# soham2560/MPCHoloNavigation

Measured on AMD Instinct MI355X. Metric: rollouts/sec per computeVelocityCommands() tick, higher is better.
Workload: dtype f32

## Files before the change

### mpcholonavigation_amd/csrc/smpc_lane.hip

```cpp

#include <hip/hip_runtime.h>
#include <stdint.h>
#include <stdio.h>

#include <type_traits>

#include "smpc_dev.h"
#include "smpc_device_math.h"
#include "smpc_tail.h"
#include "smpc_lane_common.h"
#include "smpc_inst.h"

#ifndef WAVE
#define WAVE 64
#endif
#ifndef LANE_X_RR_NOLOAD
#define LANE_X_RR_NOLOAD 0
#endif
#define LANE_BLOCK 512
#ifndef LANE_BLOCK_RR
#define LANE_BLOCK_RR 512
#endif

#ifndef LANE_X_GAMMA_N
#define LANE_X_GAMMA_N 0
#endif
#ifndef LANE_X_GAMMA_UC
#define LANE_X_GAMMA_UC 1
#endif
#ifndef LANE_X_FURTHEST_WINDOW
#define LANE_X_FURTHEST_WINDOW 1
#endif
#ifndef LANE_X_PFW_MIN
#define LANE_X_PFW_MIN 1
#endif
#ifndef LANE_X_CELL_AX
#define LANE_X_CELL_AX 1
#endif
#ifndef LANE_X_PIN_LDS
#define LANE_X_PIN_LDS 0
#endif
#ifndef LANE_X_PARK_STEP
#define LANE_X_PARK_STEP 0
#endif
#ifndef LANE_X_CONST_VGPR
#define LANE_X_CONST_VGPR 0
#endif

template <bool TO_GM>
__global__ void __launch_bounds__(256) smpc_relayout(const float* __restrict__ src, float* __restrict__ dst,
                                                    uint32_t B, uint32_t T)
{
  __shared__ float tile[32][33];
  const uint32_t b0 = blockIdx.x * 32, t0 = blockIdx.y * 32;
  const uint32_t lx = threadIdx.x & 31, ly = threadIdx.x >> 5;
  if (TO_GM) {
    for (uint32_t k = ly; k < 32; k += 8) {
      const uint32_t b = b0 + k, t = t0 + lx;
      tile[k][lx] = (b < B && t < T) ? src[(size_t)b * T + t] : 0.f;
    }
    __syncthreads();
    for (uint32_t k = ly; k < 32; k += 8) {
      const uint32_t t = t0 + k, b = b0 + lx;
      if (b < B && t < T) dst[SMPC_GM_INDEX(b, t, T)] = tile[lx][k];
    }
  } else {
    for (uint32_t k = ly; k < 32; k += 8) {
      const uint32_t t = t0 + k, b = b0 + lx;
      tile[lx][k] = (b < B && t < T) ? src[SMPC_GM_INDEX(b, t, T)] : 0.f;
    }
    __syncthreads();
    for (uint32_t k = ly; k < 32; k += 8) {
      const uint32_t b = b0 + k, t = t0 + lx;
      if (b < B && t < T) dst[(size_t)b * T + t] = tile[k][lx];
    }
  }
}

hipError_t smpc_launch_relayout(const float* src, float* dst, uint32_t B, uint32_t T, bool to_gm, hipStream_t st)
{
  const dim3 grid((B + 31) / 32, (T + 31) / 32);
  if (to_gm) hipLaunchKernelGGL(smpc_relayout<true>, grid, dim3(256), 0, st, src, dst, B, T);
  else hipLaunchKernelGGL(smpc_relayout<false>, grid, dim3(256), 0, st, src, dst, B, T);
  return hipGetLastError();
}

__global__ void __launch_bounds__(64) smpc_lane_reduce_kernel(const float* __restrict__ v,
                                                              const float* __restrict__ w,
                                                              float* __restrict__ out)
{
  const int lane = threadIdx.x;
  float V[64];
#pragma unroll
  for (int t = 0; t < 64; ++t) V[t] = v[lane * 64 + t];
  const LaneW lw = lane_weights(w[lane], lane);
  out[lane] = lane_reduce64(V, lw, lane);
}

hipError_t smpc_launch_lane_reduce(const float* v, const float* w, float* out, hipStream_t st)
{
  hipLaunchKernelGGL(smpc_lane_reduce_kernel, dim3(1), dim3(64), 0, st, v, w, out);
  return hipGetLastError();
}

#define LANE_PASS_KERNEL smpc_pass_lane
#define LANE_PASS_POW false
#include "smpc_lane_pass.inc"
#undef LANE_PASS_KERNEL
#undef LANE_PASS_POW
#define LANE_PASS_KERNEL smpc_pass_lane_pow
#define LANE_PASS_POW true
#include "smpc_lane_pass.inc"
#undef LANE_PASS_KERNEL
#undef LANE_PASS_POW

#define LANE_INST(...) {__VA_ARGS__, reinterpret_cast<const void*>(&smpc_pass_lane<__VA_ARGS__>), false}
#define LANE_INST_POW(...) {__VA_ARGS__, reinterpret_cast<const void*>(&smpc_pass_lane_pow<__VA_ARGS__>), true}
static const LaneInst kLaneInst[] = {
  LANE_INST(false, false, false, 1, false, false, false, 0, false),
  LANE_INST(true, false, false, 1, false, false, true, 0, false),
  LANE_INST(false, true, false, 1, false, false, false, 0, false),
  LANE_INST(true, true, false, 1, false, false, true, 0, false),
  LANE_INST(false, true, false, 1, false, false, true, 0, false),
  LANE_INST(false, true, false, 1, false, false, true, 56, false),
  LANE_INST(false, false, true, 1, false, false, false, 0, false),
  LANE_INST(true, false, true, 1, false, false, true, 0, false),
  LANE_INST(false, true, true, 1, false, false, false, 0, false),
  LANE_INST(true, true, true, 1, false, false, true, 0, false),
  LANE_INST(true, true, false, 1, true, false, true, 0, false),
  LANE_INST(true, true, false, 2, true, false, true, 0, false),
  LANE_INST(false, true, false, 1, false, true, false, 0, false),
  LANE_INST(true, true, false, 1, false, true, true, 0, false),
  LANE_INST(true, true, false, 1, false, false, true, 0, true),
  LANE_INST(false, true, false, 1, false, false, true, 56, true),
  LANE_INST(true, true, true, 1, false, false, true, 0, true),
  LANE_INST(false, true, true, 1, false, false, true, 56, true),
  LANE_INST_POW(true, true, false, 1, false, false, true, 0, false),
  LANE_INST_POW(false, true, false, 1, false, false, true, 0, false),
  LANE_INST_POW(false, true, false, 1, false, false, true, 56, false),
  LANE_INST_POW(false, true, false, 1, false, false, false, 0, false),
  LANE_INST_POW(true, true, false, 1, false, true, true, 0, false),
  LANE_INST_POW(false, true, false, 1, false, true, false, 0, false),
  LANE_INST_POW(true, false, false, 1, false, false, true, 0, false),
  LANE_INST_POW(false, false, false, 1, false, false, false, 0, false),
};
#undef LANE_INST
#undef LANE_INST_POW

static const LaneInst* lane_find(bool full, bool obst, bool many, int nch, bool rr, bool ga, bool quads, int tc, bool dep,
                                 bool pow = false)
{
  for (const LaneInst& k : kLaneInst)
    if (k.full == full && k.obst == obst && k.many == many && k.nch == nch && k.rr == rr && k.ga == ga &&
        k.quads == quads && k.tc == tc && k.dep == dep && k.pow == pow)
      return &k;
  return nullptr;
}

const LaneInst* lane_select(uint32_t flags, uint32_t T, bool rr, bool many, float acker_r, bool pow)
{
  const uint32_t dep_set = SD_CONSTRAINT | SD_COST | SD_TWIRLING, lean_extra = dep_set | SD_GOAL | SD_PATH_ANGLE;
  if (flags & (SD_STORE_TRAJ | SD_USE_PATH_YAW | (SD_EXTRA_CRITICS & ~lean_extra))) return nullptr;
  const bool obst = (flags & (SD_OBSTACLES | SD_COST)) != 0;
  const bool full = T == 64u;
  if (pow) {
    if (rr || many || T > 64u || (flags & lean_extra)) return nullptr;
    if (flags & SD_GOAL_ANGLE) return obst ? lane_find(full, true, false, 1, false, true, full, 0, false, true) : nullptr;
    if (obst && T == 56u) return lane_find(false, true, false, 1, false, false, true, 56, false, true);
    return lane_find(full, obst, false, 1, false, false, full || (obst && (T & 3u) == 0u), 0, false, true);
  }
  if (rr) {
    if (!(flags & SD_OBSTACLES) || (flags & (lean_extra | SD_GOAL_ANGLE)) || (T != 64u && T != 128u)) return nullptr;
    return lane_find(true, true, many, T > 64u ? 2 : 1, true, false, true, 0, false);
  }
  if (T > 64u) return nullptr;
  if (flags & dep_set) {
    if (!obst || (flags & (SD_GOAL_ANGLE | SD_GOAL)) || ((flags & SD_COST) && (flags & SD_OBSTACLES)) ||
        acker_r >= 0.f || (!full && T != 56u))
      return nullptr;
    return lane_find(full, true, many, 1, false, false, true, full ? 0 : 56, true);
  }
  if (flags & (SD_GOAL | SD_PATH_ANGLE)) return nullptr;
  if (flags & SD_GOAL_ANGLE)
    return obst ? lane_find(full, true, many, 1, false, true, full, 0, false) : nullptr;
  if (many) return lane_find(full, obst, true, 1, false, false, full, 0, false);
  if (obst && T == 56u) return lane_find(false, true, false, 1, false, false, true, 56, false);
  return lane_find(full, obst, false, 1, false, false, full || (obst && (T & 3u) == 0u), 0, false);
}

const LaneInst* lane_occupancy_row(uint32_t T, bool rr)
{
  if (rr) return lane_find(true, true, false, T > 64u ? 2 : 1, true, false, true, 0, false);
  return lane_find(T == 64u, true, false, 1, false, false, T == 64u, 0, false);
}

hipError_t lane_launch(const LaneInst* k, const SmpcDev& p, const SmpcDev* d_many, uint32_t n, const SmpcLds& L,
                       uint32_t grid, uint32_t block, hipStream_t st)
{
  if (!k || k->many != (d_many != nullptr)) return hipErrorInvalidValue;
  if (k->rr ? block != LANE_BLOCK_RR : (block != LANE_BLOCK && block != LANE_BLOCK / 2)) return hipErrorInvalidValue;
  auto b = [](bool v) {return v ? "true" : "false";};
  snprintf(smpc_last_pass_kernel, sizeof(smpc_last_pass_kernel), "smpc_pass_lane%s<%s, %s, %s, %d, %s, %s, %s, %d, %s>",
           k->pow ? "_pow" : "", b(k->full), b(k->obst), b(k->many), k->nch, b(k->rr), b(k->ga), b(k->quads), k->tc, b(k->dep));
  static const SmpcDev none{};
  void* args[] = {const_cast<SmpcDev*>(d_many ? &none : &p), const_cast<SmpcLds*>(&L), &d_many};
  return inst_launch(k->fn, d_many ? dim3(grid, n) : dim3(grid), block, args, L.total, st);
}

uint32_t smpc_lane_block() {return LANE_BLOCK;}
uint32_t smpc_lane_block_rr() {return LANE_BLOCK_RR;}

hipError_t lane_set_lds_limit(int bytes) {return inst_set_lds_limit(kLaneInst, bytes);}
```

### mpcholonavigation_amd/csrc/smpc_lane_common.h

```cpp
#ifndef SMPC_LANE_COMMON_H_
#define SMPC_LANE_COMMON_H_

#include <hip/hip_runtime.h>
#include <stdint.h>

#include "smpc_dev.h"
#include "smpc_device_math.h"

#ifndef WAVE
#define WAVE 64
#endif

typedef unsigned u32x2 __attribute__((ext_vector_type(2)));
typedef const float __attribute__((address_space(4))) * cfloat_p;
typedef float f32x32 __attribute__((ext_vector_type(32)));
typedef float f32x4 __attribute__((ext_vector_type(4)));
typedef float f32x2 __attribute__((ext_vector_type(2)));
#define LANE_PARK_STRIDE 68

struct LaneW {
  float wa, wb;
};

#define SMPC_DPP_NODE(NAME, CTRL, BANKS)                                                    \
  __device__ __forceinline__ float NAME(float a, float b)                                   \
  {                                                                                         \
    float t;                                                                                \
    asm("s_nop 1\n\t"                                                              \
                 "v_add_f32_dpp %0, %1, %1 " CTRL " row_mask:0xf bank_mask:0xf\n\t"         \
                 "v_add_f32_dpp %0, %2, %2 " CTRL " row_mask:0xf bank_mask:" BANKS          \
                 : "=&v"(t)                                                                 \
                 : "v"(a), "v"(b));                                                         \
    return t;                                                                               \
  }
SMPC_DPP_NODE(node_bit3, "row_ror:8", "0xc")
SMPC_DPP_NODE(node_bit2, "row_half_mirror", "0xa")

template <int CTRL>
__device__ __forceinline__ float dpp_mov(float v)
{
  return __uint_as_float(
    (uint32_t)__builtin_amdgcn_update_dpp(0, (int)__float_as_uint(v), CTRL, 0xF, 0xF, false));
}

template <int K, int Rr>
__device__ __forceinline__ float lane_reduce_node(const float (&V)[64], const LaneW& w, int lane)
{
  if constexpr (K == 0) {
    return V[Rr];
  } else {
    const float a = lane_reduce_node<K - 1, Rr>(V, w, lane);
    const float b = lane_reduce_node<K - 1, Rr + (64 >> K)>(V, w, lane);
    if constexpr (K == 1) {
      const u32x2 s = __builtin_amdgcn_permlane32_swap(__float_as_uint(a), __float_as_uint(b),
                                                       false, false);
      return fmaf(w.wa, __uint_as_float(s.x), w.wb * __uint_as_float(s.y));
    } else if constexpr (K == 2) {
      const u32x2 s = __builtin_amdgcn_permlane16_swap(__float_as_uint(a), __float_as_uint(b),
                                                       false, false);
      return __uint_as_float(s.x) + __uint_as_float(s.y);
    } else if constexpr (K == 3) {
      return node_bit3(a, b);
    } else if constexpr (K == 4) {
      return node_bit2(a, b);
    } else if constexpr (K == 5) {
      const float ta = a + dpp_mov<0x4E>(a);
      const float tb = b + dpp_mov<0x4E>(b);
      return (lane & 2) ? tb : ta;
    } else {
      const float ta = a + dpp_mov<0xB1>(a);
      const float tb = b + dpp_mov<0xB1>(b);
      return (lane & 1) ? tb : ta;
    }
  }
}

__device__ __forceinline__ LaneW lane_weights(float w, int lane)
{
  const float wo = __shfl_xor(w, 32, WAVE);
  LaneW r;
  r.wa = lane < 32 ? w : wo;
  r.wb = lane < 32 ? wo : w;
  return r;
}

__device__ __forceinline__ float lane_reduce64(const float (&V)[64], const LaneW& w, int lane)
{
  return lane_reduce_node<6, 0>(V, w, lane);
}

__device__ __forceinline__ int cvt_floor_i32(float q)
{
  int r;
  asm("v_cvt_flr_i32_f32 %0, %1" : "=v"(r) : "v"(q));
  return r;
}

__device__ __forceinline__ uint32_t cell_byte_exact(const SmpcDev& p, uint8_t* s_map, float x,
                                                    float y, uint32_t slot)
{
  const uint32_t nwin = (uint32_t)(p.win_w * p.win_h);
  uint32_t mx = 0, my = 0;
  bool on = cell_index_exact((double)x, p.ox, p.res, p.W, mx);
  on = cell_index_exact((double)y, p.oy, p.res, p.H, my) && on;
  if (!on) return nwin;
  const uint32_t wx = mx - (uint32_t)p.win_x0, wy = my - (uint32_t)p.win_y0;
  if (wx < (uint32_t)p.win_w && wy < (uint32_t)p.win_h) return wy * p.win_w + wx;
  s_map[nwin + 1 + slot] = p.map[(size_t)my * p.W + mx];
  return nwin + 1 + slot;
}

#endif
```

### mpcholonavigation_amd/csrc/smpc_lane_pass.inc

```
template <bool FULL, bool OBST, bool MANY, int NCH, bool RR, bool GA = false, bool QUADS = FULL, int TC = 0, bool DEP = false>
__global__ void __launch_bounds__(RR ? LANE_BLOCK_RR : LANE_BLOCK, (RR && LANE_BLOCK_RR == 256) ? 3 : 1)
LANE_PASS_KERNEL(const SmpcDev p0, const SmpcLds L, const SmpcDev* __restrict__ many)
{
  constexpr bool POW = LANE_PASS_POW;
  static_assert(RR || NCH == 1, "parked controls: one chunk of 64 steps");
  static_assert(!POW || (!MANY && !RR && !DEP), "cost powers: the single-context parking form of the five critics");
  static_assert(!FULL || QUADS, "T == 64 is a multiple of four");
  static_assert(TC == 0 || (!FULL && QUADS && !RR && TC < 64 && (TC & 3) == 0), "compile-time horizon: whole quads below 64");
  static_assert(!DEP || (OBST && !RR && !GA), "deployed-list instances: parking form");
  const SmpcDev& p = MANY ? many[blockIdx.y] : p0;
  const SmpcTickPtrs tk{p.u, p.px, p.py, p.pyaw, p.D, p.pf_idx, p.pvalid, p.pa_active, p.pang_active, p.pal_active};
  extern __shared__ __attribute__((aligned(16))) unsigned char smem[];
  uint8_t* s_map = smem;
  const SmpcLut* s_lut = reinterpret_cast<const SmpcLut*>(smem + L.off_lut);
  float* s_px = reinterpret_cast<float*>(smem + L.off_px);
  float* s_py = reinterpret_cast<float*>(smem + L.off_py);
  float* s_D = reinterpret_cast<float*>(smem + L.off_D) + 1;
  f32x4* s_pts4 = reinterpret_cast<f32x4*>(smem + L.off_pts4);
  float* s_su2 = reinterpret_cast<float*>(smem + L.off_scr) - 4;

  constexpr int BLK = RR ? LANE_BLOCK_RR : LANE_BLOCK;
  const int blk = blockDim.x;
  const int tid = threadIdx.x;
  const int lane = tid & (WAVE - 1);
  const int wave = __builtin_amdgcn_readfirstlane(tid >> 6);
  const int nwave = blockDim.x >> 6;
  auto stamp = [&](int k) {
    if (__builtin_expect(p.timeline != nullptr, 0) && tid == 0)
      p.timeline[blockIdx.x * 8 + k] = __builtin_amdgcn_s_memtime();
  };
  stamp(0);
  float* park = reinterpret_cast<float*>(smem + L.off_scr) + (size_t)wave * L.scr_stride;
  float* s_w = park + 64 * LANE_PARK_STRIDE;

  {
    const int ww = OBST ? p.win_w : 0, wh = OBST ? p.win_h : 0;
    const bool vec = OBST && ((ww & 3) == 0) && ((p.W & 3u) == 0) && ((p.win_x0 & 3) == 0);
    const int w4 = OBST ? (ww >> 2) : 1, n4 = vec ? w4 * wh : 0;
    auto word = [&](int i) -> uint32_t {
      const int ry = i / w4, rx = i - ry * w4;
      return reinterpret_cast<const uint32_t*>(p.map + (size_t)(p.win_y0 + ry) * p.W + p.win_x0)[rx];
    };
    constexpr int kAhead = 96 * 96 / 4 / BLK + 1;
    uint32_t tmp[kAhead];
#pragma unroll
    for (int k = 0; k < kAhead; ++k) {
      const int i = tid + k * blk;
      tmp[k] = i < n4 ? word(i) : 0u;
    }
    const SmpcLut lut_e = (OBST && tid < 256) ? p.lut[tid] : SmpcLut{0.f, 0.f};
    const bool pt_on = (uint32_t)tid < p.P, seg_on = (uint32_t)tid + 1 < p.P;
    const float g_px = pt_on ? tk.px[tid] : 0.f, g_py = pt_on ? tk.py[tid] : 0.f;
    const float g_D = seg_on ? tk.D[tid] : 0.f;
    const bool g_valid = seg_on && tk.pvalid[tid] != 0;

    if (OBST) {
#pragma unroll
      for (int k = 0; k < kAhead; ++k) {
        const int i = tid + k * blk;
        if (i < n4) reinterpret_cast<uint32_t*>(s_map)[i] = tmp[k];
      }
      for (int i = tid + kAhead * blk; i < n4; i += blk)
        reinterpret_cast<uint32_t*>(s_map)[i] = word(i);
      if (!vec) {
        for (int i = tid; i < ww * wh; i += blockDim.x) {
          const int ry = i / ww, rx = i - ry * ww;
          s_map[i] = p.map[(size_t)(p.win_y0 + ry) * p.W + p.win_x0 + rx];
        }
      }
      if (tid < 256) const_cast<SmpcLut*>(s_lut)[tid] = lut_e;
      if (tid == 0) const_cast<SmpcLut*>(s_lut)[256] = SmpcLut{0.f, 0.f};
      if (tid == 0) s_map[ww * wh] = 255;
    }
    for (uint32_t i = p.P + tid; i < ((p.P + 3u) & ~3u); i += blockDim.x) s_px[i] = s_py[i] = 1.0e18f;
    if (pt_on) {
      s_px[tid] = g_px;
      s_py[tid] = g_py;
      if (seg_on) s_D[tid] = g_D;
      s_pts4[tid] = f32x4{g_px, g_py, g_valid ? 1.0f : 0.f, 0.f};
    }
#if LANE_X_GAMMA_UC
    if (tid < WAVE) {
      float a = 0.f, b = 0.f, c = 0.f;
      const uint32_t Tn = FULL ? 64u * NCH : (TC ? (uint32_t)TC : p.T);
      for (uint32_t t = (uint32_t)tid; t < Tn; t += WAVE) {
        const float ux = tk.u[t], uy = tk.u[Tn + t], uz = tk.u[2 * Tn + t];
        a = fmaf(ux, ux, a);
        b = fmaf(uy, uy, b);
        c = fmaf(uz, uz, c);
      }
      for (int o = 32; o > 0; o >>= 1) {
        a += __shfl_xor(a, o, WAVE);
        b += __shfl_xor(b, o, WAVE);
        c += __shfl_xor(c, o, WAVE);
      }
      if (tid == 0) {
        s_su2[0] = a;
        s_su2[1] = b;
        s_su2[2] = c;
      }
    }
#endif
    for (uint32_t i = tid + blk; i < p.P; i += blk) {
      const float qx = tk.px[i], qy = tk.py[i];
      const bool seg = i + 1 < p.P;
      s_px[i] = qx;
      s_py[i] = qy;
      if (seg) s_D[i] = tk.D[i];
      s_pts4[i] = f32x4{qx, qy, (seg && tk.pvalid[i]) ? 1.0f : 0.f, 0.f};
    }
  }
  __syncthreads();
  stamp(1);

  const cfloat_p cu = (cfloat_p)(uintptr_t)p.u;
  const uint32_t T = FULL ? 64u * NCH : (TC ? (uint32_t)TC : p.T), B = p.B;
  const uint32_t noise_bytes = T * SMPC_GM_ROLLOUTS(B) * 4u;
  const __amdgpu_buffer_rsrc_t rn = __builtin_amdgcn_make_buffer_rsrc(const_cast<float*>(p.tvx), 0, 3u * noise_bytes, 0x00020000);
  const float dt = p.dt, yaw0 = p.yaw0;
  const double x0 = p.x0, y0 = p.y0;
  uint32_t S = 0;
  if (p.flags & SD_NEED_FURTHEST) {
    S = p.d_furthest ? smpc_furthest_index(*p.d_furthest) : p.furthest_hint;
    if (S >= p.P) S = p.P ? p.P - 1 : 0;
  }
  if (lane == 0) {
    s_D[-1] = -3.0e38f;
    s_D[S] = 3.0e38f;
  }
  const bool pa_on = (p.flags & SD_PATH_ALIGN) && p.P > 0 && tk.pa_active[S] && S > 0;
  float pf_x = 0.f, pf_y = 0.f;
  if ((p.flags & SD_PATH_FOLLOW) && p.P > 0) {
    const uint32_t idx = tk.pf_idx[S];
    pf_x = tk.px[idx];
    pf_y = tk.py[idx];
  }
  const uint32_t bs_iters = S > 1 ? 32u - (uint32_t)__builtin_clz(S - 1) : 0u;
  float pa_inv_spacing = 0.f;
  if (pa_on && S > 1 && tk.D[S - 1] > 0.f) pa_inv_spacing = (float)(S - 1) / tk.D[S - 1];
  const bool want_local_furthest = (p.flags & SD_NEED_FURTHEST) && (p.flags & SD_LOCAL_FURTHEST);
  const bool con_on = DEP && (p.flags & SD_CONSTRAINT) != 0, tw_on = DEP && (p.flags & SD_TWIRLING) != 0;
  const float k_con = p.dt * p.con_weight, k_tw = p.tw_weight / (float)(FULL ? 64 * NCH : (TC ? TC : (int)p.T));
  const bool cost_mode = DEP && (p.flags & SD_COST) != 0;
  constexpr bool ga_on = GA;
  const uint32_t nquad = (T + 3u) >> 2;

  float m_run = 3.0e38f, s_run = 0.f;
  float Ux[NCH], Uy[NCH], Uz[NCH];
#pragma unroll
  for (int h = 0; h < NCH; ++h) Ux[h] = Uy[h] = Uz[h] = 0.f;
  float F_local = 0.f;
  uint32_t n_noncoll = 0;

  const uint32_t ngroups = (B + WAVE - 1) / WAVE;
  const uint32_t gw = blockIdx.x * nwave + wave;
  const uint32_t nW = gridDim.x * nwave;

  auto group_body = [&](auto safe_c, const uint32_t grp) -> bool {
    constexpr bool SAFE = decltype(safe_c)::value;
    const uint32_t b = grp * WAVE + lane;
    const bool live = b < B;
    const uint32_t bl = live ? b : B - 1;
    f32x32 PX0, PX1, PY0, PY1;
    if (!FULL && !RR) PX0 = PX1 = PY0 = PY1 = (f32x32)(0.f);

    float cpx = p.svx, cpy = p.svy, cpz = p.swz;
    float acc_yaw = 0.f, ax = 0.f, ay = 0.f;
    float cs_prev = p.cos0, sn_prev = p.sin0;
    float x = 0.f, y = 0.f;
    float crit = 0.f, rep = 0.f;
    float yaw_max = 0.f;
    float alive = 1.0f;
    uint32_t cell_q = 256u;
    f32x2 e_q = {0.f, 0.f};
    [[maybe_unused]] const uint32_t lds_lut = (uint32_t)(uintptr_t)s_lut, lds_map = (uint32_t)(uintptr_t)s_map;
    auto lookup_wait = [&]() {
#if LANE_X_PIN_LDS
      asm volatile("s_waitcnt lgkmcnt(0)" : "+v"(cell_q), "+v"(e_q));
#endif
    };
    auto lookup_accumulate = [&]() {
      alive = e_q.x < 0.f ? 0.f : alive;
      crit = fmaf(alive, e_q.x, crit);
      rep = fmaf(alive, e_q.y, rep);
    };
#if LANE_X_PIN_LDS
    auto lookup_issue_entry = [&]() {
      const uint32_t a = lds_lut + (cell_q << 3);
      asm volatile("ds_read_b64 %0, %1" : "=v"(e_q) : "v"(a));
    };
    auto lookup_issue_byte = [&](uint32_t idx) {
      const uint32_t a = lds_map + idx;
      asm volatile("ds_read_u8 %0, %1" : "=v"(cell_q) : "v"(a));
    };
#else
    auto lookup_issue_entry = [&]() {
      const SmpcLut e = s_lut[cell_q];
      e_q = f32x2{e.crit, e.rep};
    };
    auto lookup_issue_byte = [&](uint32_t idx) {cell_q = s_map[idx];};
#endif
    float pfw = 0.f, gx = 0.f, gy = 0.f, gz = 0.f;
    float ga_sum = 0.f;
    float ext = 0.f;
    float traj_dist = 0.f, pa_sum = 0.f, pa_num = 0.f, sx_prev = p.x00f, sy_prev = p.y00f;
    uint32_t path_pt = 0;

#if LANE_X_CONST_VGPR
    const float k_rinv = in_vgpr(p.rinvf), k_cx = in_vgpr(p.cxf), k_cy = in_vgpr(p.cyf);
#else
    const float k_rinv = p.rinvf, k_cx = p.cxf, k_cy = p.cyf;
#endif
    const float k_edge = 0.5f - p.cell_eps_w;
    auto do_step = [&](const uint32_t t, const bool sample_slot, const float ux, const float uy, const float uz,
                       const float n0, const float n1, const float n2, float& cvx, float& cvy,
                       float& cwz) {
      cvx = ux + n0;
      cvy = uy + n1;
      cwz = uz + n2;
      const float vx = cpx, vy = cpy, wz = cpz;
      cpx = cvx;
      cpy = cvy;
      cpz = cwz;
      acc_yaw = acc_yaw + wz * dt;
      const float yaw = acc_yaw + yaw0;
      const float dxr = vx * cs_prev - vy * sn_prev;
      const float dyr = vx * sn_prev + vy * cs_prev;
      ax = ax + dxr * dt;
      ay = ay + dyr * dt;
      if constexpr (DEP) {
        if (con_on) {
          const float sp = fast_sqrt(vx * vx + vy * vy);
          const float vt = vx > 0.f ? sp : -sp;
          const float e = fmaxf(vt - p.con_max_vel, 0.f) + fmaxf(p.con_min_vel - vt, 0.f);
          ext = fmaf(e, k_con, ext);
        }
        if (tw_on) ext = fmaf(fabsf(wz), k_tw, ext);
      }
      if (ga_on) {
        const float a = p.ga_goal_yaw - yaw;
        const float kf = fmaf(a, 0.15915494309189535f, 12582912.0f);
        const float k = kf - 12582912.0f;
        float r = fmaf(-k, 6.2831854820251465f, a);
        r = fmaf(-k, -1.7484555e-07f, r);
        ga_sum += fabsf(r);
      }

      uint32_t idx = 0;
      if (OBST) {
#if LANE_X_CELL_AX
        const float qx = fmaf(ax, k_rinv, k_cx), qy = fmaf(ay, k_rinv, k_cy);
#else
        x = (float)(x0 + (double)ax);
        y = (float)(y0 + (double)ay);
        const float qx = (x - p.wxf) * p.rinvf, qy = (y - p.wyf) * p.rinvf;
#endif
        const float rx = __builtin_amdgcn_fractf(qx), ry = __builtin_amdgcn_fractf(qy);
        const int lx = cvt_floor_i32(qx), ly = cvt_floor_i32(qy);
        const float edge = fmaxf(fabsf(rx - 0.5f), fabsf(ry - 0.5f));
        const bool fast = (edge <= k_edge) &
                          ((uint32_t)lx < (uint32_t)p.win_w) & ((uint32_t)ly < (uint32_t)p.win_h);
        idx = __umul24((uint32_t)ly, (uint32_t)p.win_w) + (uint32_t)lx;
        if (__builtin_expect(__builtin_amdgcn_ballot_w64(!fast) != 0, 0)) {
          if (!fast)
            idx = cell_byte_exact(p, s_map, (float)(x0 + (double)ax), (float)(y0 + (double)ay),
                                  (uint32_t)(wave * WAVE + lane));
        }
      }

      if (SAFE) {
        smpc_sincos(yaw, sn_prev, cs_prev);
      } else {
        yaw_max = fmaxf(yaw_max, fabsf(yaw));
        smpc_sincos_fast(yaw, sn_prev, cs_prev);
      }
#if LANE_X_PFW_MIN
      pfw = pfw + fminf(vx, 0.f);
#else
      pfw = fmaf(fmaxf(-vx, 0.f), dt, pfw);
#endif
#if LANE_X_GAMMA_UC
      gx = fmaf(ux, cvx, gx);
      gz = fmaf(uz, cwz, gz);
      gy = fmaf(uy, cvy, gy);
#elif LANE_X_GAMMA_N
      gx = fmaf(ux, n0, gx);
      gz = fmaf(uz, n2, gz);
      gy = fmaf(uy, n1, gy);
#else
      gx = fmaf(ux, cvx - ux, gx);
      gz = fmaf(uz, cwz - uz, gz);
      gy = fmaf(uy, cvy - uy, gy);
#endif

      if (sample_slot && pa_on && t != 0) {
        x = (float)(x0 + (double)ax);
        y = (float)(y0 + (double)ay);
        const float ddx = x - sx_prev, ddy = y - sy_prev;
        traj_dist += fast_sqrt(ddx * ddx + ddy * ddy);
        sx_prev = x;
        sy_prev = y;
        const float dist = traj_dist;
        uint32_t gi = (uint32_t)(dist * pa_inv_spacing);
        gi = gi < S ? gi : S - 1;
        const float da = s_D[(int)gi - 1];
        const float db = s_D[gi];
        const float dc = s_D[gi + 1];
        const bool c0 = da < dist, c1 = db < dist, c2 = dc < dist;
        uint32_t lo = gi + (c1 ? 1u : 0u);
        float dl = c1 ? db : da, dh = c1 ? dc : db;
        if (__builtin_expect(__builtin_amdgcn_ballot_w64(!c0 || c2) != 0, 0)) {
          uint32_t base = 0, nn = S;
          for (uint32_t it = 0; it < bs_iters; ++it) {
            const uint32_t half = nn >> 1;
            base = (s_D[base + half - 1 + (half == 0)] < dist && half) ? base + half : base;
            nn -= half;
          }
          const float d_base = s_D[base];
          lo = base + (d_base < dist ? 1u : 0u);
          dl = lo > 0 ? s_D[lo - 1] : 0.f;
          dh = lo < S ? s_D[lo] : 0.f;
        }
        uint32_t pt;
        if (lo == path_pt) pt = 0;
        else if (lo >= S) pt = S - 1;
        else pt = (dist - dl < dh - dist) ? lo - 1 : lo;
        path_pt = pt;
        const f32x4 q = s_pts4[pt];
        const float ex = q[0] - x, ey = q[1] - y;
        const float d = fast_sqrt(ex * ex + ey * ey);
        pa_num += q[2];
        pa_sum = fmaf(q[2], d, pa_sum);
      }
      if (OBST) {
        lookup_wait();
        lookup_accumulate();
        lookup_issue_entry();
        lookup_issue_byte(idx);
      }
    };

    const uint32_t loff = ((bl >> 6) * T * 64u + (bl & 63u)) * 4u;
    constexpr uint32_t step_bytes = 256u;
    auto ld = [&](uint32_t tensor, uint32_t t) -> float {
      const uint32_t tc = (FULL || t < T) ? t : T - 1;
      return __uint_as_float(__builtin_amdgcn_raw_buffer_load_b32(rn, loff, tensor * noise_bytes + tc * step_bytes, 0));
    };
    auto ldu = [&](uint32_t ctrl, uint32_t t) -> float {return cu[ctrl * T + ((FULL || t < T) ? t : T - 1)];};
    float nq[12], uq[12];
#pragma unroll
    for (int i = 0; i < 4; ++i) {
      nq[3 * i + 0] = ld(0, i);
      nq[3 * i + 1] = ld(1, i);
      nq[3 * i + 2] = ld(2, i);
#pragma unroll
      for (int k = 0; k < 3; ++k) uq[3 * i + k] = ldu(k, i);
    }
    uint64_t clk = __builtin_amdgcn_s_memtime();
    auto run_quad = [&](auto hi_c, const uint32_t q, float (&cq)[12]) {
      [[maybe_unused]] constexpr bool HI = decltype(hi_c)::value;
      if (((uint32_t)(clk >> 15) + (uint32_t)(wave >> 2)) & 1u) __builtin_amdgcn_s_setprio(1);
      else __builtin_amdgcn_s_setprio(0);
      clk = __builtin_amdgcn_s_memtime();
      float uc[12];
#pragma unroll
      for (int j = 0; j < 12; ++j) uc[j] = uq[j];
      constexpr bool kAlwaysAhead = !FULL && TC == 0;
      if (kAlwaysAhead || q + 1 < nquad) {
#pragma unroll
        for (int i = 0; i < 4; ++i)
#pragma unroll
          for (int k = 0; k < 3; ++k) uq[3 * i + k] = ldu(k, 4 * (q + 1) + i);
      }
#pragma unroll
      for (int i = 0; i < 4; ++i) {
        const uint32_t t = 4 * q + i;
        const float n0 = nq[3 * i], n1 = nq[3 * i + 1], n2 = nq[3 * i + 2];
        if (kAlwaysAhead || q + 1 < nquad) {
          nq[3 * i + 0] = ld(0, t + 4);
          nq[3 * i + 1] = ld(1, t + 4);
          nq[3 * i + 2] = ld(2, t + 4);
        }
        cq[3 * i] = cq[3 * i + 1] = cq[3 * i + 2] = 0.f;
        if (QUADS || t < T)
          do_step(t, i == 0, uc[3 * i], uc[3 * i + 1], uc[3 * i + 2], n0, n1, n2, cq[3 * i], cq[3 * i + 1],
                  cq[3 * i + 2]);
#if LANE_X_PARK_STEP
        if constexpr (RR) {
        } else if constexpr (HI) {
          PX1[8 * i + (q - 8)] = cq[3 * i];
          PY1[8 * i + (q - 8)] = cq[3 * i + 1];
        } else {
          PX0[8 * i + q] = cq[3 * i];
          PY0[8 * i + q] = cq[3 * i + 1];
        }
        if constexpr (!RR) park[(4 * q + i) * LANE_PARK_STRIDE + lane] = cq[3 * i + 2];
#endif
      }
    };
    if constexpr (RR) {
#pragma unroll 2
      for (uint32_t q = 0; q < nquad; ++q) {
        float cq[12];
        run_quad(std::false_type{}, q, cq);
      }
    } else {
      const uint32_t qh = nquad < 8u ? nquad : 8u;
      if constexpr (QUADS && !FULL && TC == 0) {
        auto quad_lo = [&](const uint32_t q) {
          float cq[12];
          run_quad(std::false_type{}, q, cq);
#if !LANE_X_PARK_STEP
#pragma unroll
          for (int i = 0; i < 4; ++i) {
            PX0[8 * i + q] = cq[3 * i];
            PY0[8 * i + q] = cq[3 * i + 1];
            park[(4 * q + i) * LANE_PARK_STRIDE + lane] = cq[3 * i + 2];
          }
#endif
        };
        auto quad_hi = [&](const uint32_t q) {
          float cq[12];
          run_quad(std::true_type{}, q, cq);
#if !LANE_X_PARK_STEP
#pragma unroll
          for (int i = 0; i < 4; ++i) {
            PX1[8 * i + (q - 8)] = cq[3 * i];
            PY1[8 * i + (q - 8)] = cq[3 * i + 1];
            park[(4 * q + i) * LANE_PARK_STRIDE + lane] = cq[3 * i + 2];
          }
#endif
        };
        uint32_t q = 0;
        for (; q + 1 < qh; q += 2) {
          quad_lo(q);
          quad_lo(q + 1);
        }
        if (q < qh) quad_lo(q);
        q = 8;
        for (; q + 1 < nquad; q += 2) {
          quad_hi(q);
          quad_hi(q + 1);
        }
        if (q < nquad) quad_hi(q);
      } else {
#pragma unroll 2
        for (uint32_t q = 0; q < qh; ++q) {
          float cq[12];
          run_quad(std::false_type{}, q, cq);
#if !LANE_X_PARK_STEP
#pragma unroll
          for (int i = 0; i < 4; ++i) {
            PX0[8 * i + q] = cq[3 * i];
            PY0[8 * i + q] = cq[3 * i + 1];
            park[(4 * q + i) * LANE_PARK_STRIDE + lane] = cq[3 * i + 2];
          }
#endif
        }
#pragma unroll 2
        for (uint32_t q = 8; q < nquad; ++q) {
          float cq[12];
          run_quad(std::true_type{}, q, cq);
#if !LANE_X_PARK_STEP
#pragma unroll
          for (int i = 0; i < 4; ++i) {
            PX1[8 * i + (q - 8)] = cq[3 * i];
            PY1[8 * i + (q - 8)] = cq[3 * i + 1];
            park[(4 * q + i) * LANE_PARK_STRIDE + lane] = cq[3 * i + 2];
          }
#endif
        }
      }
    }
    if (OBST) {
      lookup_wait();
      lookup_accumulate();
      lookup_issue_entry();
      lookup_wait();
      lookup_accumulate();
    }
    if (!SAFE && __builtin_expect(__any(!(yaw_max < 65536.0f) || !(fabsf(acc_yaw) < 65536.0f)), 0)) return true;

    x = (float)(x0 + (double)ax);
    y = (float)(y0 + (double)ay);

    if (want_local_furthest) {
      auto block_d2 = [&](const float* bx, const float* by, float (&dd)[4]) {
        const f32x4 qx = *reinterpret_cast<const f32x4*>(bx);
        const f32x4 qy = *reinterpret_cast<const f32x4*>(by);
#pragma unroll
        for (int e = 0; e < 4; ++e) {
          const float ex = qx[e] - x, ey = qy[e] - y;
          dd[e] = ex * ex + ey * ey;
        }
      };
      float best = 3.4028234663852886e38f;
      uint32_t bj = 0;
      const uint32_t P4 = (p.P + 3u) & ~3u;
      constexpr bool kWindow = LANE_X_FURTHEST_WINDOW && !GA && !DEP && !MANY;
      const uint32_t j_lo = (kWindow && (S >> 2) > 3u) ? ((S >> 2) - 3u) << 2 : 0u;
      for (uint32_t j = j_lo; j < P4; j += 4) {
        float dd[4];
        block_d2(s_px + j, s_py + j, dd);
        const float mn = fminf(fminf(dd[0], dd[1]), fminf(dd[2], dd[3]));
        if (mn < best) {
          best = mn;
          bj = j;
        }
      }
      auto point_F = [&]() -> float {
        float dd[4];
        block_d2(s_px + bj, s_py + bj, dd);
        const uint32_t bi = bj + (dd[0] == best ? 0u : dd[1] == best ? 1u : dd[2] == best ? 2u : dd[3] == best ? 3u : 0u);
        float F = (float)bi;
        if (bi + 1 < p.P) {
          const float nx = s_px[bi + 1], ny = s_py[bi + 1];
          const float sgx = nx - s_px[bi], sgy = ny - s_py[bi];
          const float d_next = (nx - x) * (nx - x) + (ny - y) * (ny - y);
          const float seg2 = sgx * sgx + sgy * sgy;
          const float tt = seg2 > 0.f ? 0.5f + 0.5f * (best - d_next) * fast_rcp(seg2) : 0.f;
          F = fmaxf(F + fminf(fmaxf(tt, -0.45f), 0.45f), 0.f);
        }
        return F;
      };
      float F = point_F();
      float m = live ? F : 0.f;
      for (int o = 32; o > 0; o >>= 1) m = fmaxf(m, __shfl_xor(m, o, WAVE));
      if (kWindow && j_lo) {
        const unsigned long long holders = __ballot(live && F == m);
        bool below = false;
        if (holders) {
          const int wl = __builtin_ctzll(holders);
          const float wx = __shfl(x, wl, WAVE), wy = __shfl(y, wl, WAVE), wbest = __shfl(best, wl, WAVE);
          for (uint32_t k = (uint32_t)lane; k < j_lo; k += WAVE) {
            const float ex = s_px[k] - wx, ey = s_py[k] - wy;
            below = below || (ex * ex + ey * ey <= wbest);
          }
        }
        if (__builtin_expect(__any(below), 0)) {
          for (uint32_t jj = j_lo; jj > 0; jj -= 4) {
            const uint32_t j = jj - 4;
            float dd[4];
            block_d2(s_px + j, s_py + j, dd);
            const float mn = fminf(fminf(dd[0], dd[1]), fminf(dd[2], dd[3]));
            if (mn <= best) {
              best = mn;
              bj = j;
            }
          }
          F = point_F();
          m = live ? F : 0.f;
          for (int o = 32; o > 0; o >>= 1) m = fmaxf(m, __shfl_xor(m, o, WAVE));
        }
      }
      F_local = fmaxf(F_local, m);
    }
    float cost = (p.flags & SD_ACCUMULATE) ? p.costs_prev[bl] : 0.f;
    if constexpr (POW) {
      if (OBST) {
        const bool collided = alive == 0.f;
        const float raw = collided ? p.obs_collision_cost : crit;
        const float v = (p.obs_critical_w * raw) + (p.obs_repulsion_w * rep / (float)T);
        cost = add_cost_pow(cost, (double)v, p.obs_power);
        n_noncoll += (uint32_t)__popcll(__ballot(live && !collided));
      }
      if (pa_on) {
        const float c_pa = pa_num > 0.f ? pa_sum / pa_num : 0.f;
        cost = add_cost_pow(cost, (double)(c_pa * p.pa_weight), p.pa_power);
      }
      if (p.flags & SD_PATH_FOLLOW) {
        const double ddx = (double)(x - pf_x), ddy = (double)(y - pf_y);
        cost = add_cost_pow(cost, (double)in_vgpr(p.pf_weight) * sqrt_unscaled(ddx * ddx + ddy * ddy), p.pf_power);
      }
      if (ga_on) {
        const double Td = (FULL || TC) ? (double)T : (double)in_vgpr((float)T);
        cost = add_cost_pow(cost, (double)ga_sum / Td * (double)in_vgpr(p.ga_weight), p.ga_power);
      }
#if LANE_X_PFW_MIN
      if (p.flags & SD_PREFER_FORWARD) cost = add_cost_pow(cost, (double)((pfw * -dt) * p.pfw_weight), p.pfw_power);
#else
      if (p.flags & SD_PREFER_FORWARD) cost = add_cost_pow(cost, (double)(pfw * p.pfw_weight), p.pfw_power);
#endif
#if LANE_X_GAMMA_UC
      cost += p.g_vx * (gx - s_su2[0]);
      cost += p.g_wz * (gz - s_su2[2]);
      cost += p.g_vy * (gy - s_su2[1]);
#else
      cost += p.g_vx * gx;
      cost += p.g_wz * gz;
      cost += p.g_vy * gy;
#endif
    } else {
      float lin = 0.f, uni = 0.f;
      if (OBST) {
        const bool collided = alive == 0.f;
        if (cost_mode) {
          const float k = p.cost_w254 / (float)T;
          lin = collided ? 0.f : k * rep;
          uni = collided ? k * p.cost_collision_cost : 0.f;
        } else {
          lin = (collided ? 0.f : p.obs_critical_w * crit) + p.obs_rep_over_T * rep;
          uni = collided ? p.obs_critical_w * p.obs_collision_cost : 0.f;
        }
        n_noncoll += (uint32_t)__popcll(__ballot(live && !collided));
      }
      if constexpr (DEP) lin += ext;
      if (p.flags & SD_PATH_FOLLOW) {
        const float fdx = x - pf_x, fdy = y - pf_y;
        uni += p.pf_weight * fast_sqrt(fdx * fdx + fdy * fdy);
      }
#if LANE_X_PFW_MIN
      if (p.flags & SD_PREFER_FORWARD) lin += (pfw * -dt) * p.pfw_weight;
#else
      if (p.flags & SD_PREFER_FORWARD) lin += pfw * p.pfw_weight;
#endif
      if (ga_on) uni += (ga_sum / (float)T) * p.ga_weight;
#if LANE_X_GAMMA_UC
      lin += p.g_vx * (gx - s_su2[0]);
      lin += p.g_wz * (gz - s_su2[2]);
      lin += p.g_vy * (gy - s_su2[1]);
#else
      lin += p.g_vx * gx;
      lin += p.g_wz * gz;
      lin += p.g_vy * gy;
#endif
      cost += uni + lin;
      if (pa_on) {
        const float c_pa = pa_num > 0.f ? pa_sum * fast_rcp(pa_num) : 0.f;
        cost += c_pa * p.pa_weight;
      }
    }
    if (live) p.costs[b] = cost;

    float cmin = live ? cost : 3.0e38f;
    for (int o = 32; o > 0; o >>= 1) cmin = fminf(cmin, __shfl_xor(cmin, o, WAVE));
    const float m_new = fminf(m_run, cmin);
    const float f = __builtin_amdgcn_exp2f(p.k2 * (m_run - m_new));
    const float w = live ? __builtin_amdgcn_exp2f(p.k2 * (cost - m_new)) : 0.f;
    float wsum = w;
    for (int o = 32; o > 0; o >>= 1) wsum += __shfl_xor(wsum, o, WAVE);
    s_run = fmaf(s_run, f, wsum);
    m_run = m_new;

    const LaneW lw = lane_weights(w, lane);
    if constexpr (RR) {
#pragma unroll
      for (int h = 0; h < NCH; ++h) {
#pragma unroll
        for (int ctrl = 0; ctrl < 3; ++ctrl) {
          float V[64];
#pragma unroll
          for (int t = 0; t < 64; ++t) V[t] = LANE_X_RR_NOLOAD ? (float)t : ld(ctrl, 64u * h + t);
          __builtin_amdgcn_sched_barrier(0);
#pragma unroll
          for (int t = 0; t < 64; ++t) {
            const uint32_t tt = 64u * h + t;
            const float c = ldu(ctrl, tt) + V[t];
            V[t] = (FULL || tt < T) ? c : 0.f;
          }
          const float r = lane_reduce64(V, lw, lane);
          if (ctrl == 0) Ux[h] = fmaf(Ux[h], f, r);
          else if (ctrl == 1) Uy[h] = fmaf(Uy[h], f, r);
          else Uz[h] = fmaf(Uz[h], f, r);
        }
      }
    } else {
      {
        float V[64];
#pragma unroll
        for (int t = 0; t < 32; ++t) {
          V[t] = PX0[8 * (t & 3) + (t >> 2)];
          V[32 + t] = PX1[8 * (t & 3) + (t >> 2)];
        }
        Ux[0] = fmaf(Ux[0], f, lane_reduce64(V, lw, lane));
#pragma unroll
        for (int t = 0; t < 32; ++t) {
          V[t] = PY0[8 * (t & 3) + (t >> 2)];
          V[32 + t] = PY1[8 * (t & 3) + (t >> 2)];
        }
        Uy[0] = fmaf(Uy[0], f, lane_reduce64(V, lw, lane));
      }
      {
        s_w[lane] = w;
        __builtin_amdgcn_fence(__ATOMIC_RELEASE, "wavefront");
        __builtin_amdgcn_wave_barrier();
        __builtin_amdgcn_fence(__ATOMIC_ACQUIRE, "wavefront");
        const f32x4* row = reinterpret_cast<const f32x4*>(park + lane * LANE_PARK_STRIDE);
        float acc0 = 0.f, acc1 = 0.f;
#pragma unroll
        for (int bq = 0; bq < 16; bq += 2) {
          const f32x4 w0 = reinterpret_cast<const f32x4*>(s_w)[bq], c0 = row[bq];
          const f32x4 w1 = reinterpret_cast<const f32x4*>(s_w)[bq + 1], c1 = row[bq + 1];
#pragma unroll
          for (int e = 0; e < 4; ++e) {
            acc0 = fmaf(w0[e], c0[e], acc0);
            acc1 = fmaf(w1[e], c1[e], acc1);
          }
        }
        Uz[0] = fmaf(Uz[0], f, acc0 + acc1);
        __builtin_amdgcn_wave_barrier();
      }
    }
    return false;
  };

  stamp(2);
  int stamp_k = 3;
  for (uint32_t grp = gw; grp < ngroups; grp += nW) {
    if (__builtin_expect(group_body(std::false_type{}, grp), 0)) group_body(std::true_type{}, grp);
    if (stamp_k < 5) stamp(stamp_k++);
  }

  if (__builtin_expect(p.timeline != nullptr, 0) && lane == 0)
    p.timeline[8192 + blockIdx.x * 8 + wave] = __builtin_amdgcn_s_memtime();
  __syncthreads();
  stamp(5);
  const uint32_t TL = 4 + 3 * T;
  float* myp = reinterpret_cast<float*>(smem + L.off_scr) + (size_t)wave * L.scr_stride;
  if (lane == 0) {
    myp[0] = m_run;
    myp[1] = s_run;
    myp[2] = F_local;
    myp[3] = (float)n_noncoll;
  }
#pragma unroll
  for (int h = 0; h < NCH; ++h) {
    const uint32_t tt = 64u * h + (uint32_t)lane;
    if (tt < T) {
      myp[4 + tt] = Ux[h];
      myp[4 + T + tt] = Uy[h];
      myp[4 + 2 * T + tt] = Uz[h];
    }
  }
  __syncthreads();
  const float* allp = reinterpret_cast<const float*>(smem + L.off_scr);
  float bm = 3.0e38f;
  for (int w = 0; w < nwave; ++w) bm = fminf(bm, allp[(size_t)w * L.scr_stride]);
  float* outp = p.partials + (size_t)blockIdx.x * TL;
  for (uint32_t i = tid; i < TL; i += blockDim.x) {
    float acc = 0.f;
    if (i == 0) {
      acc = bm;
    } else if (i == 2) {
      for (int w = 0; w < nwave; ++w) acc = fmaxf(acc, allp[(size_t)w * L.scr_stride + 2]);
    } else if (i == 3) {
      for (int w = 0; w < nwave; ++w) acc += allp[(size_t)w * L.scr_stride + 3];
    } else {
      for (int w = 0; w < nwave; ++w) {
        const float mw = allp[(size_t)w * L.scr_stride];
        const float sc = __builtin_amdgcn_exp2f(p.k2 * (mw - bm));
        acc += sc * allp[(size_t)w * L.scr_stride + i];
      }
    }
    smpc_store_partial(outp + i, acc);
  }
  stamp(6);
  if (!(p.flags & SD_ACCUMULATE) && blockIdx.x == 0 && tid == 0) outp[SMPC_CANARY_SLOT(T)] = cu[-4];
  if constexpr (!MANY && !RR) {
    if (p.tail) smpc_grid_tail<(RR ? LANE_BLOCK_RR : LANE_BLOCK) / 64>(p, smem);
  }
}
```

Baseline: 5.287 billion.

## Pair quad iterations with per-pair priority swap, quad-offset noise loads, inline-asm min-add

Adds three default-on knobs to the lane pass kernel. The forward-progress accumulation becomes a two-instruction inline asm (v_min_f32 then v_add_f32). For full or fixed-T quad paths, the loop is unrolled in pairs and s_setprio/s_memtime run only on the first quad of each pair. Noise prefetch loads use precomputed per-quad scalar offsets on the buffer load instead of the generic ld() helper. The aim is less scalar and address overhead per step, at the cost of coarser priority switching between waves and more code size.

```diff
diff --git a/mpcholonavigation_amd/csrc/smpc_lane.hip b/mpcholonavigation_amd/csrc/smpc_lane.hip
--- a/mpcholonavigation_amd/csrc/smpc_lane.hip
+++ b/mpcholonavigation_amd/csrc/smpc_lane.hip
@@ -45,6 +45,16 @@
 #endif
 #ifndef LANE_X_CONST_VGPR
 #define LANE_X_CONST_VGPR 0
+#endif
+
+#ifndef LANE_X_PFW_BARE
+#define LANE_X_PFW_BARE 1
+#endif
+#ifndef LANE_X_NOISE_QUAD
+#define LANE_X_NOISE_QUAD 1
+#endif
+#ifndef LANE_X_PRIO_ITER
+#define LANE_X_PRIO_ITER 1
 #endif
 
 template <bool TO_GM>
diff --git a/mpcholonavigation_amd/csrc/smpc_lane_common.h b/mpcholonavigation_amd/csrc/smpc_lane_common.h
--- a/mpcholonavigation_amd/csrc/smpc_lane_common.h
+++ b/mpcholonavigation_amd/csrc/smpc_lane_common.h
@@ -96,6 +96,13 @@
   return r;
 }
 
+__device__ __forceinline__ float add_min_zero(float acc, float x)
+{
+  float m;
+  asm("v_min_f32 %1, 0, %2\n\tv_add_f32 %0, %0, %1" : "+v"(acc), "=&v"(m) : "v"(x));
+  return acc;
+}
+
 __device__ __forceinline__ uint32_t cell_byte_exact(const SmpcDev& p, uint8_t* s_map, float x,
                                                     float y, uint32_t slot)
 {
diff --git a/mpcholonavigation_amd/csrc/smpc_lane_pass.inc b/mpcholonavigation_amd/csrc/smpc_lane_pass.inc
--- a/mpcholonavigation_amd/csrc/smpc_lane_pass.inc
+++ b/mpcholonavigation_amd/csrc/smpc_lane_pass.inc
@@ -156,6 +156,8 @@
   const uint32_t gw = blockIdx.x * nwave + wave;
   const uint32_t nW = gridDim.x * nwave;
 
+  using T_ = std::true_type;
+  using F_ = std::false_type;
   auto group_body = [&](auto safe_c, const uint32_t grp) -> bool {
     constexpr bool SAFE = decltype(safe_c)::value;
     const uint32_t b = grp * WAVE + lane;
@@ -214,7 +216,7 @@
     const float k_edge = 0.5f - p.cell_eps_w;
     auto do_step = [&](const uint32_t t, const bool sample_slot, const float ux, const float uy, const float uz,
                        const float n0, const float n1, const float n2, float& cvx, float& cvy,
-                       float& cwz) {
+                       float& cwz) __attribute__((always_inline)) {
       cvx = ux + n0;
       cvy = uy + n1;
       cwz = uz + n2;
@@ -274,7 +276,9 @@
         yaw_max = fmaxf(yaw_max, fabsf(yaw));
         smpc_sincos_fast(yaw, sn_prev, cs_prev);
       }
-#if LANE_X_PFW_MIN
+#if LANE_X_PFW_MIN && LANE_X_PFW_BARE
+      pfw = add_min_zero(pfw, vx);
+#elif LANE_X_PFW_MIN
       pfw = pfw + fminf(vx, 0.f);
 #else
       pfw = fmaf(fmaxf(-vx, 0.f), dt, pfw);
@@ -357,11 +361,19 @@
       for (int k = 0; k < 3; ++k) uq[3 * i + k] = ldu(k, i);
     }
     uint64_t clk = __builtin_amdgcn_s_memtime();
-    auto run_quad = [&](auto hi_c, const uint32_t q, float (&cq)[12]) {
+    auto run_quad = [&](auto hi_c, auto swap_c, const uint32_t q, float (&cq)[12]) __attribute__((always_inline)) {
       [[maybe_unused]] constexpr bool HI = decltype(hi_c)::value;
-      if (((uint32_t)(clk >> 15) + (uint32_t)(wave >> 2)) & 1u) __builtin_amdgcn_s_setprio(1);
-      else __builtin_amdgcn_s_setprio(0);
-      clk = __builtin_amdgcn_s_memtime();
+      constexpr bool SWAP = decltype(swap_c)::value;
+      if constexpr (SWAP) {
+#if LANE_X_PRIO_ITER
+        __builtin_amdgcn_s_setprio(0);
+        if (((uint32_t)(clk >> 15) + (uint32_t)(wave >> 2)) & 1u) __builtin_amdgcn_s_setprio(1);
+#else
+        if (((uint32_t)(clk >> 15) + (uint32_t)(wave >> 2)) & 1u) __builtin_amdgcn_s_setprio(1);
+        else __builtin_amdgcn_s_setprio(0);
+#endif
+        clk = __builtin_amdgcn_s_memtime();
+      }
       float uc[12];
 #pragma unroll
       for (int j = 0; j < 12; ++j) uc[j] = uq[j];
@@ -372,14 +384,26 @@
 #pragma unroll
           for (int k = 0; k < 3; ++k) uq[3 * i + k] = ldu(k, 4 * (q + 1) + i);
       }
+      constexpr bool kQuadOff = LANE_X_NOISE_QUAD && QUADS && !GA && !DEP && !MANY && !POW;
 #pragma unroll
       for (int i = 0; i < 4; ++i) {
         const uint32_t t = 4 * q + i;
         const float n0 = nq[3 * i], n1 = nq[3 * i + 1], n2 = nq[3 * i + 2];
         if (kAlwaysAhead || q + 1 < nquad) {
-          nq[3 * i + 0] = ld(0, t + 4);
-          nq[3 * i + 1] = ld(1, t + 4);
-          nq[3 * i + 2] = ld(2, t + 4);
+          if constexpr (kQuadOff) {
+            const uint32_t tq = (FULL || TC || 4 * (q + 1) < T) ? 4 * (q + 1) : T - 4;
+            const uint32_t so0 = tq * step_bytes, so1 = noise_bytes + so0, so2 = noise_bytes + so1;
+            auto ldq = [&](uint32_t so) -> float {
+              return __uint_as_float(__builtin_amdgcn_raw_buffer_load_b32(rn, loff + (uint32_t)i * step_bytes, so, 0));
+            };
+            nq[3 * i + 0] = ldq(so0);
+            nq[3 * i + 1] = ldq(so1);
+            nq[3 * i + 2] = ldq(so2);
+          } else {
+            nq[3 * i + 0] = ld(0, t + 4);
+            nq[3 * i + 1] = ld(1, t + 4);
+            nq[3 * i + 2] = ld(2, t + 4);
+          }
         }
         cq[3 * i] = cq[3 * i + 1] = cq[3 * i + 2] = 0.f;
         if (QUADS || t < T)
@@ -398,18 +422,62 @@
 #endif
       }
     };
+    constexpr bool kPairLoops = LANE_X_PRIO_ITER && (FULL || TC != 0);
+    if constexpr (kPairLoops) {
+#if LANE_X_PARK_STEP
+#define LANE_PARK_QUAD(HI, Q)
+#else
+#define LANE_PARK_QUAD(HI, Q) \
+      if constexpr (!RR) { \
+        _Pragma("unroll") for (int i = 0; i < 4; ++i) { \
+          if constexpr (HI) { \
+            PX1[8 * i + ((Q) - 8)] = cq[3 * i]; \
+            PY1[8 * i + ((Q) - 8)] = cq[3 * i + 1]; \
+          } else { \
+            PX0[8 * i + (Q)] = cq[3 * i]; \
+            PY0[8 * i + (Q)] = cq[3 * i + 1]; \
+          } \
+          park[(4 * (Q) + i) * LANE_PARK_STRIDE + lane] = cq[3 * i + 2]; \
+        } \
+      }
+#endif
+#define LANE_QUAD(HI, SWAP, Q) \
+    { \
+      float cq[12]; \
+      run_quad(std::bool_constant<HI>{}, std::bool_constant<SWAP>{}, (Q), cq); \
+      LANE_PARK_QUAD(HI, Q) \
+    }
+#define LANE_QUADS(HI, Q0, QE)    \
+    { \
+      uint32_t q = (Q0); \
+      const uint32_t qe = (QE); \
+      for (; q + 1 < qe; q += 2) { \
+        LANE_QUAD(HI, true, q) \
+        LANE_QUAD(HI, false, q + 1) \
+      } \
+      if (q < qe) LANE_QUAD(HI, true, q) \
+    }
     if constexpr (RR) {
+      LANE_QUADS(false, 0u, nquad)
+    } else {
+      LANE_QUADS(false, 0u, nquad < 8u ? nquad : 8u)
+      LANE_QUADS(true, 8u, nquad)
+    }
+#undef LANE_QUADS
+#undef LANE_QUAD
+#undef LANE_PARK_QUAD
+    } else if constexpr (RR) {
 #pragma unroll 2
       for (uint32_t q = 0; q < nquad; ++q) {
         float cq[12];
-        run_quad(std::false_type{}, q, cq);
+        run_quad(F_{}, T_{}, q, cq);
       }
     } else {
       const uint32_t qh = nquad < 8u ? nquad : 8u;
       if constexpr (QUADS && !FULL && TC == 0) {
         auto quad_lo = [&](const uint32_t q) {
           float cq[12];
-          run_quad(std::false_type{}, q, cq);
+          run_quad(F_{}, T_{}, q, cq);
 #if !LANE_X_PARK_STEP
 #pragma unroll
           for (int i = 0; i < 4; ++i) {
@@ -421,7 +489,7 @@
         };
         auto quad_hi = [&](const uint32_t q) {
           float cq[12];
-          run_quad(std::true_type{}, q, cq);
+          run_quad(T_{}, T_{}, q, cq);
 #if !LANE_X_PARK_STEP
 #pragma unroll
           for (int i = 0; i < 4; ++i) {
@@ -447,7 +515,7 @@
 #pragma unroll 2
         for (uint32_t q = 0; q < qh; ++q) {
           float cq[12];
-          run_quad(std::false_type{}, q, cq);
+          run_quad(F_{}, T_{}, q, cq);
 #if !LANE_X_PARK_STEP
 #pragma unroll
           for (int i = 0; i < 4; ++i) {
@@ -460,7 +528,7 @@
 #pragma unroll 2
         for (uint32_t q = 8; q < nquad; ++q) {
           float cq[12];
-          run_quad(std::true_type{}, q, cq);
+          run_quad(T_{}, T_{}, q, cq);
 #if !LANE_X_PARK_STEP
 #pragma unroll
           for (int i = 0; i < 4; ++i) {
@@ -707,7 +775,7 @@
   stamp(2);
   int stamp_k = 3;
   for (uint32_t grp = gw; grp < ngroups; grp += nW) {
-    if (__builtin_expect(group_body(std::false_type{}, grp), 0)) group_body(std::true_type{}, grp);
+    if (__builtin_expect(group_body(F_{}, grp), 0)) group_body(T_{}, grp);
     if (stamp_k < 5) stamp(stamp_k++);
   }
 
```

Result: faster. 5.419 billion, median of 6 (+2.5%).
